# mahyarnajibi/SNIPER

Hardware: AMD Instinct MI355X
Metric: train chips/sec (512x512, R101) (higher is better)
Workload: dtype f16

## Files before the change

include/sniper_hip.h:

```cpp
#ifndef SNIPER_HIP_H
#define SNIPER_HIP_H

#include <stddef.h>
#include <stdint.h>

#ifdef __cplusplus
extern "C" {
#endif

typedef void *sn_stream_t;

enum { SN_OK = 0, SN_ERR_ARG = 1, SN_ERR_HIP = 2, SN_ERR_WORKSPACE = 3, SN_ERR_UNSUPPORTED = 4 };

int sn_version(void);
const char *sn_last_error(void);
int sn_debug_option(const char *name, int value);

int sn_iou_f64(const double *d_boxes, int N, const double *d_query, int K, double *d_out, int mode, sn_stream_t stream);

int sn_chips_num_candidates(int width, int height, int chipsize, int stride);
size_t sn_chips_workspace_bytes(int total_cand, int max_boxes_per_unit);
int sn_chips_generate_batch(const float *d_boxes, const int32_t *d_box_off, const int32_t *d_meta, const int32_t *d_perm,
                            const int32_t *d_cand_off, int U, int max_boxes_per_unit, void *d_mask_ws, float *d_out_chips,
                            int32_t *d_out_ids, int32_t *d_out_count, sn_stream_t stream);
// ... 11 lines not shown

int sn_focus_mask(const float *d_gt, const int32_t *d_ngt, const double *d_crop, const float *d_scale, int B, int G, int F,
                  int feat_stride, int im_h, int im_w, float dc_low, float small_thresh, float dc_high, float *d_mask,
                  sn_stream_t stream);

size_t sn_nms_workspace_bytes(int B, int N);
int sn_nms_batch(const float *d_boxes, const int32_t *d_n, int B, int N, int dim, float thresh, int max_keep, void *d_ws,
                 int32_t *d_keep, int32_t *d_nkeep, sn_stream_t stream);
int sn_nms_host(int *keep_out, int *num_out, const float *boxes_host, int boxes_num, int boxes_dim,
                float nms_overlap_thresh, int device_id);

size_t sn_soft_nms_max_boxes(void);
size_t sn_soft_nms_workspace_bytes(size_t total_rows);
int sn_soft_nms_batch(float *d_boxes, const int32_t *d_off, int P, int max_n, size_t total_rows, float sigma, float Nt,
                      float threshold, int method, void *d_ws, int32_t *d_count, sn_stream_t stream);

int sn_im_prepare(const uint8_t *d_src_bgr, int src_h, int src_w, int crop_x1, int crop_y1, int crop_x2, int crop_y2, double scale,
                  int flip, const double *pixel_means_bgr3, float *d_out, int out_h, int out_w, int32_t *resized_hw2,
                  sn_stream_t stream);
int sn_bbox_decode(const float *d_rois, const float *d_deltas, const float *d_im_info, double *d_boxes, int B, int R,
                   sn_stream_t stream);
int sn_focus_rects_host(const uint8_t *mask_hw, int H, int W, int mode, int32_t *rects_xywh, int cap, int32_t *n_rects);
int sn_focus_chips_host(const float *map_hw, int H, int W, int d, float thresh, int ms, double im_width, double im_height,
                        double cscale, double *chips_xyxy, int max_chips, int32_t *n_chips);
int sn_aggregate_problems_host(const uint64_t *part_rows, const int64_t *lens, const int32_t *part_of_image, const float *range2,
                               int P, int nc, int num_images, float *out_rows, long capacity_rows, int64_t *out_sizes,
                               int64_t *total_rows);
int sn_aggregate_count(const void *d_parts, int P, int nc, int32_t *d_kept, sn_stream_t stream);
int sn_aggregate_scatter(const void *d_parts, int P, int nc, const int32_t *d_dst_off, float *d_out_rows, sn_stream_t stream);
int sn_det_cap_per_image(float *d_rows, const int32_t *d_off, int32_t *d_count, int num_images, int nc, int max_per_image,
                         sn_stream_t stream);
int sn_det_compact(const float *d_scores, const double *d_boxes, const double *h_crops, const double *h_im_wh, float thresh,
                   double delta, int B, int R, int NC, double *d_rows, int32_t *d_counts, sn_stream_t stream);


int sn_conv_fwd(const void *x, const void *w, const float *bias, const void *residual, void *y, int N, int H, int W, int Cin,
                int in_pix_stride, int Cout, int out_pix_stride, int res_pix_stride, int KH, int KW, int stride, int pad, int dil,
                int relu, int out_f32, sn_stream_t stream);
size_t sn_conv_fwd_splitk_workspace_bytes(int N, int H, int W, int Cin, int in_pix_stride, int Cout, int out_pix_stride,
                                          int res_pix_stride, int KH, int KW, int stride, int pad, int dil);
int sn_conv_fwd_splitk(const void *x, const void *w, const float *bias, const void *residual, void *y, int N, int H, int W, int Cin,
                       int in_pix_stride, int Cout, int out_pix_stride, int res_pix_stride, int KH, int KW, int stride, int pad,
                       int dil, int relu, void *ws, size_t ws_bytes, sn_stream_t stream);
int sn_conv_fwd_splitk_f32(const void *x, const void *w, const float *bias, float *y, int N, int H, int W, int Cin, int in_pix_stride,
                           int Cout, int out_pix_stride, int KH, int KW, int stride, int pad, int dil, int relu, void *ws,
                           size_t ws_bytes, sn_stream_t stream);
int sn_conv_fwd_dual_ok(int N, int H, int W, int Cin, int in_pix_stride, int Cout, int out_pix_stride, int res_pix_stride, int KH,
                        int KW, int stride, int pad, int dil, int y2_pix_stride);
int sn_conv_fwd_dual(const void *x, const void *w, const float *bias, const void *residual, void *y, int N, int H, int W, int Cin,
                     int in_pix_stride, int Cout, int out_pix_stride, int res_pix_stride, int KH, int KW, int stride, int pad, int dil,
                     int relu, void *y2, int y2_pix_stride, const float *y2_scale, const float *y2_shift, int y2_relu, void *ws,
                     size_t ws_bytes, sn_stream_t stream);
int sn_conv_tune(int cfg);

int sn_conv_fwd_stats_blocks(int N, int H, int W, int Cin, int in_pix_stride, int Cout, int out_pix_stride, int res_pix_stride,
                             int KH, int KW, int stride, int pad, int dil);
int sn_conv_fwd_stats(const void *x, const void *w, const float *bias, const void *residual, void *y, int N, int H, int W, int Cin,
                      int in_pix_stride, int Cout, int out_pix_stride, int res_pix_stride, int KH, int KW, int stride, int pad,
                      int dil, int relu, float *stats, sn_stream_t stream);
int sn_conv_stem_fwd(const void *xp, const void *w, const float *bias, void *y, int N, int Hp, int Wp, int Ho, int Wo, int Cout,
                     int out_pix_stride, int KH, int KWP, int stride, int relu, int out_f32, sn_stream_t stream);
size_t sn_conv_stem_wgrad_workspace_bytes(int N, int Ho, int Wo, int Cout, int KH, int KWP);
int sn_conv_stem_wgrad(const void *dy, const void *xp, float *dw, int N, int Hp, int Wp, int Ho, int Wo, int Cout, int dy_pix_stride,
                       int KH, int KWP, int stride, void *ws, size_t ws_bytes, sn_stream_t stream);
int sn_conv_dgrad(const void *dy, const void *wt, const void *accumulate, void *dx, int N, int H, int W, int Cin,
                  int dx_pix_stride, int Cout, int dy_pix_stride, int acc_pix_stride, int KH, int KW, int stride, int pad, int dil,
                  int out_f32, sn_stream_t stream);
int sn_conv_dgrad_by_class(int on);
int sn_conv_dgrad_bn_blocks(int N, int H, int W, int Cin, int dx_pix_stride, int Cout, int dy_pix_stride, int acc_pix_stride, int KH,
                            int KW, int stride, int pad, int dil);
int sn_conv_dgrad_bn(const void *dy, const void *wt, const void *accumulate, void *dx, int N, int H, int W, int Cin, int dx_pix_stride,
                     int Cout, int dy_pix_stride, int acc_pix_stride, int KH, int KW, int stride, int pad, int dil, const void *bn_x,
                     int bn_x_pix_stride, const float *bn_scale, const float *bn_shift, const float *bn_mean, int bn_act,
                     float *partials, sn_stream_t stream);
size_t sn_conv_wgrad_workspace_bytes(int N, int H, int W, int Cin, int x_pix_stride, int Cout, int dy_pix_stride, int KH, int KW,
                                     int stride, int pad, int dil);
int sn_conv_wgrad(const void *dy, const void *x, float *dw, int N, int H, int W, int Cin, int x_pix_stride, int Cout,
                  int dy_pix_stride, int KH, int KW, int stride, int pad, int dil, void *ws, size_t ws_bytes, sn_stream_t stream);
typedef struct sn_wgrad_desc {
  const void *dy, *x;
  float *dw;
  int N, H, W, Cin, x_pix_stride, Cout, dy_pix_stride, KH, KW, stride, pad, dil;
} sn_wgrad_desc;
size_t sn_conv_wgrad_batch_workspace_bytes(const sn_wgrad_desc *descs, int n);
int sn_conv_wgrad_batch(const sn_wgrad_desc *descs, int n, void *ws, size_t ws_bytes, sn_stream_t stream);
int sn_conv_wgrad_impl(int impl, int job_steps);
int sn_conv_wgrad_trace(void *buf);
int sn_conv_trace(void *buf);
size_t sn_bias_grad_workspace_bytes(long rows, int C);
int sn_bias_grad(const void *dy, float *db, long rows, int C, int ld, int dtype, void *ws, size_t ws_bytes, sn_stream_t stream);

int sn_pack_stem_input(const float *x_nchw, void *out, int N, int C, int H, int W, int Hp, int Wp, int pad_t, int pad_l,
                       const float *scale, const float *shift, sn_stream_t stream);

size_t sn_bn_workspace_bytes(int M, int C);
int sn_bn_stats(const void *x, int M, int C, int ps, void *ws, sn_stream_t stream);
int sn_bn_finalize(const void *ws, int M, int C, float eps, float momentum, const float *gamma, const float *beta,
                   float *run_mean, float *run_var, float *scale, float *shift, float *save_mean, float *save_invstd,
                   sn_stream_t stream);
int sn_bn_finalize_blocks(const float *partials, int nblk, int M, int C, float eps, float momentum, const float *gamma,
                          const float *beta, float *run_mean, float *run_var, float *scale, float *shift, float *save_mean,
                          float *save_invstd, sn_stream_t stream);
int sn_bn_global_scale_shift(const float *gamma, const float *beta, const float *mean, const float *var, int C, float eps,
                             float *scale, float *shift, sn_stream_t stream);
int sn_bn_apply(const void *x, void *y, int M, int C, int ps_in, int ps_out, const float *scale, const float *shift, int relu,
                sn_stream_t stream);
// ... 253 lines not shown
```

sniper_amd/csrc/common.h:

```cpp
#pragma once
#include <hip/hip_runtime.h>
#include <stdint.h>
#include <stdio.h>
#include <stdlib.h>

#include "../../include/sniper_hip.h"

#define SN_EXPORT extern "C" __attribute__((visibility("default")))

void sn_set_error(const char *fmt, ...);

#define SN_REQUIRE(cond, ...)      \
  do {                             \
    if (!(cond)) {                 \
      sn_set_error(__VA_ARGS__);   \
      return SN_ERR_ARG;           \
    }                              \
  } while (0)

#define SN_CHECK_LAUNCH()                                                      \
  do {                                                                         \
    hipError_t e__ = hipGetLastError();                                        \
    if (e__ != hipSuccess) {                                                   \
      sn_set_error("%s:%d HIP launch failed: %s", __FILE__, __LINE__, hipGetErrorString(e__)); \
      return SN_ERR_HIP;                                                       \
    }                                                                          \
  } while (0)

#define SN_HIP(call)                                                           \
  do {                                                                         \
    hipError_t e__ = (call);                                                   \
    if (e__ != hipSuccess) {                                                   \
      sn_set_error("%s:%d %s: %s", __FILE__, __LINE__, #call, hipGetErrorString(e__)); \
      return SN_ERR_HIP;                                                       \
    }                                                                          \
  } while (0)

hipError_t sn_once_per_device_max_lds(const void *kernel, int bytes);
enum SnDebugOption { SN_OPT_PROPOSAL_FULL_SORT = 0, SN_OPT_NMS_FULL_MASK = 1, SN_OPT_CONV_NO_PERSIST = 2, SN_OPT_SOFTMAX_STRIDED = 3, SN_OPT_COUNT };
int sn_debug_get(SnDebugOption which);

static inline hipStream_t sn_stream(sn_stream_t s) { return (hipStream_t)s; }
static inline int sn_div_up(int a, int b) { return (a + b - 1) / b; }
static inline size_t sn_align(size_t x, size_t a = 256) { return (x + a - 1) / a * a; }

static inline int sn_env_int(const char *name, int dflt) {
  const char *v = getenv(name);
  return v && *v ? atoi(v) : dflt;
}
static inline int sn_conv_out(int in, int k, int stride, int pad, int dil) { return (in + 2 * pad - dil * (k - 1) - 1) / stride + 1; }
static inline int sn_blocks(long total, int cap) {
  const long b = (total + 255) / 256;
  return (int)(b < 1 ? 1 : (b > cap ? cap : b));
}

constexpr int kWave = 64;

typedef _Float16 half_t;
typedef _Float16 half8 __attribute__((ext_vector_type(8)));
typedef _Float16 half4 __attribute__((ext_vector_type(4)));
typedef float floatx4 __attribute__((ext_vector_type(4)));

__device__ __forceinline__ unsigned sn_float_key(float f) {
  const unsigned u = __float_as_uint(f);
  return (u & 0x80000000u) ? ~u : (u | 0x80000000u);
}

int sn_partial_sum(const float *part, int nblk, long n, float *dst, hipStream_t s);

struct SnDiv { unsigned mul, sh, d; };
static inline SnDiv sn_div_make(unsigned d) {
  SnDiv f;
  unsigned s = 0;
  while ((1ull << s) < d) ++s;
  f.mul = (unsigned)((((unsigned long long)1 << 32) * (((unsigned long long)1 << s) - d)) / d + 1);
  f.sh = s;
  f.d = d;
  return f;
}
__device__ __forceinline__ unsigned sn_div(unsigned n, const SnDiv f) { return (__umulhi(n, f.mul) + n) >> f.sh; }
__device__ __forceinline__ unsigned sn_divmod(unsigned n, const SnDiv f, unsigned &rem) {
  const unsigned q = sn_div(n, f);
  rem = n - q * f.d;
  return q;
}
```

sniper_amd/csrc/common.hip:

```cpp
#include "common.h"

#include <stdarg.h>
#include <stdlib.h>
#include <string.h>

#include <atomic>
#include <mutex>
#include <string>
#include <utility>
#include <vector>

static thread_local char g_err[512] = "";

void sn_set_error(const char *fmt, ...) {
  va_list ap;
  va_start(ap, fmt);
  vsnprintf(g_err, sizeof(g_err), fmt, ap);
  va_end(ap);
}

SN_EXPORT const char *sn_last_error(void) { return g_err; }
SN_EXPORT int sn_version(void) { return 100; }

hipError_t sn_once_per_device_max_lds(const void *kernel, int bytes) {
  static std::mutex mu;
  static std::vector<std::pair<const void *, int>> done;
  int dev = 0;
  hipError_t e = hipGetDevice(&dev);
  if (e != hipSuccess) return e;
  std::lock_guard<std::mutex> lock(mu);
  for (const auto &d : done)
    if (d.first == kernel && d.second == dev) return hipSuccess;
  e = hipFuncSetAttribute(kernel, hipFuncAttributeMaxDynamicSharedMemorySize, bytes);
  if (e == hipSuccess) done.emplace_back(kernel, dev);
  return e;
}

static std::atomic<int> g_debug[SN_OPT_COUNT];
static const char *const kDebugNames[SN_OPT_COUNT] = {"proposal_full_sort", "nms_full_mask", "conv_no_persist", "softmax_strided"};
static const char *const kDebugEnv[SN_OPT_COUNT] = {"SNIPER_FULL_SORT", "SNIPER_NMS_FULL", "SNIPER_CONV_NO_PERSIST", "SNIPER_SOFTMAX_STRIDED"};
namespace {
struct DebugInit {
  DebugInit() {
    for (int i = 0; i < SN_OPT_COUNT; ++i) g_debug[i].store(getenv(kDebugEnv[i]) != nullptr ? 1 : 0, std::memory_order_relaxed);
  }
} g_debug_init;
}

int sn_debug_get(SnDebugOption which) { return g_debug[which].load(std::memory_order_relaxed); }

__global__ __launch_bounds__(256) void partial_sum_kernel(const float *__restrict__ part, int nblk, long n, float *__restrict__ dst) {
  const long e = (long)blockIdx.x * 256 + threadIdx.x;
  if (e >= n) return;
  float s = 0.f;
  int k = 0;
  for (; k + 8 <= nblk; k += 8) {
    float v[8];
#pragma unroll
    for (int u = 0; u < 8; ++u) v[u] = part[(size_t)(k + u) * n + e];
#pragma unroll
    for (int u = 0; u < 8; ++u) s += v[u];
  }
  for (; k < nblk; ++k) s += part[(size_t)k * n + e];
  dst[e] += s;
}

int sn_partial_sum(const float *part, int nblk, long n, float *dst, hipStream_t s) {
  hipLaunchKernelGGL(partial_sum_kernel, dim3((unsigned)((n + 255) / 256)), dim3(256), 0, s, part, nblk, n, dst);
  SN_CHECK_LAUNCH();
  return SN_OK;
}

SN_EXPORT int sn_debug_option(const char *name, int value) {
  SN_REQUIRE(name, "sn_debug_option: null name");
  for (int i = 0; i < SN_OPT_COUNT; ++i)
    if (strcmp(name, kDebugNames[i]) == 0) {
      g_debug[i].store(value, std::memory_order_relaxed);
      return SN_OK;
    }
  SN_REQUIRE(false, "sn_debug_option: unknown option '%s'", name);
}
```

sniper_amd/csrc/conv.hip:

```cpp
#include <algorithm>
#include <atomic>

#include "conv_common.h"

#include <stdlib.h>

__device__ __forceinline__ int swz(int row, int chunk) { return chunk ^ ((0x78 >> (2 * ((row >> 2) & 3))) & 3); }

template <int BM, int BN, bool DGRAD>
__global__ __launch_bounds__(256) void conv_igemm_kernel(const ConvParams p) {
  constexpr int BK = 32;
  constexpr int WM = BM / 2, WN = BN / 2;
  constexpr int MI = WM / 16, NI = WN / 16;
  constexpr int AR = BM / 64, BR = BN / 64;
  __shared__ __attribute__((aligned(16))) half_t sA[2][BM * BK];
  __shared__ __attribute__((aligned(16))) half_t sB[2][BN * BK];

  const int tid = threadIdx.x, lane = tid & 63, wave = tid >> 6;
  const int wm = wave >> 1, wn = wave & 1;
  const int m0 = blockIdx.x * BM, n0 = blockIdx.y * BN;
  const int chunk = tid & 3, lrow = tid >> 2;

  int a_base[AR], a_h[AR], a_w[AR];
  bool a_ok[AR];
// ... 73 lines not shown
#pragma unroll
    for (int i = 0; i < MI; ++i) {
      const int r = wm * WM + i * 16 + fr;
      fa[i] = *reinterpret_cast<const half8 *>(&sA[cur][(r * 4 + swz(r, fq)) * 8]);
    }
#pragma unroll
    for (int j = 0; j < NI; ++j) {
      const int r = wn * WN + j * 16 + fr;
      fb[j] = *reinterpret_cast<const half8 *>(&sB[cur][(r * 4 + swz(r, fq)) * 8]);
    }
#pragma unroll
    for (int i = 0; i < MI; ++i)
#pragma unroll
      for (int j = 0; j < NI; ++j) acc[i][j] = __builtin_amdgcn_mfma_f32_16x16x32_f16(fa[i], fb[j], acc[i][j], 0, 0, 0);
    if (kt + 1 < nk) lstore(cur ^ 1);
    __syncthreads();
  }

#pragma unroll
  for (int i = 0; i < MI; ++i) {
#pragma unroll
    for (int r = 0; r < 4; ++r) {
      const int m = m0 + wm * WM + i * 16 + fq * 4 + r;
      if (m >= p.M) continue;
#pragma unroll
      for (int j = 0; j < NI; ++j) {
        const int n = n0 + wn * WN + j * 16 + fr;
        if (n >= p.Nout) continue;
        float v = acc[i][j][r];
        if (p.bias) v += p.bias[n];
        if (p.res) v += (float)p.res[(size_t)m * p.res_ps + n];
        if (p.relu) v = v > 0.f ? v : 0.f;
        if (p.out_f32) reinterpret_cast<float *>(p.y)[(size_t)m * p.out_ps + n] = v;
        else reinterpret_cast<half_t *>(p.y)[(size_t)m * p.out_ps + n] = (half_t)v;
      }
    }
  }
}

static int conv_check(const ConvParams &p, const char *who) {
  SN_REQUIRE(p.x && p.w && p.y, "%s: null pointer", who);
  SN_REQUIRE(p.N > 0 && p.H > 0 && p.W > 0 && p.Ho > 0 && p.Wo > 0 && p.Nout > 0, "%s: bad dims", who);
  SN_REQUIRE(p.Cin > 0 && p.Cin % 8 == 0, "%s: channels per tap must be a multiple of 8 (got %d)", who, p.Cin);
  SN_REQUIRE(p.in_ps % 8 == 0 || (p.in_ps == 4 && p.stride % 2 == 0 && p.KW == 1 && p.pad == 0 && p.W % 2 == 0),
             "%s: source pixel stride must be a multiple of 8 elements (got %d)", who, p.in_ps);
  SN_REQUIRE(p.KH > 0 && p.KW > 0 && p.stride > 0 && p.dil > 0 && p.pad >= 0, "%s: bad kernel geometry", who);
  SN_REQUIRE((long)p.N * p.H * p.W * p.in_ps < (1l << 31) && (long)p.M * p.out_ps < (1l << 31),
             "%s: tensor too large for 32-bit offsets", who);
  return SN_OK;
}

struct ConvPlan {
  int bm, mtiles, ntiles, dma;
  unsigned x_bytes, w_bytes;
  int cls, cls_mc;
};
static std::atomic<int> g_conv_cfg{sn_env_int("SNIPER_CONV_CFG", -1)};
SN_EXPORT int sn_conv_tune(int cfg) {
  SN_REQUIRE(cfg == -1 || cfg == 0 || conv_dma_config(cfg).bm > 0, "sn_conv_tune: no configuration %d", cfg);
  g_conv_cfg.store(cfg, std::memory_order_relaxed);
  return SN_OK;
}

static int conv_dma_choice_balanced(int M, int Nout, int nk, bool dgrad) {
  const long t128 = (long)sn_div_up(M, 128) * sn_div_up(Nout, 128);
  if (t128 >= 3840 && nk >= 8) return 7;
  if (Nout < 128) return nk >= 64 ? 5 : 6;
  if (M < 8192) return (Nout >= 1024 && nk >= 128) ? 4 : 6;
  const int bal = 14, bal_d = 16;
  if (nk <= 1) return 6;
  if (nk >= 16 && (long)sn_div_up(M, 160) * sn_div_up(Nout, 128) <= 320) return 18;
  return dgrad ? bal_d : bal;
}

static std::atomic<int> g_dgrad_by_class{sn_env_int("SNIPER_DGRAD_BY_CLASS", 1)};
SN_EXPORT int sn_conv_dgrad_by_class(int on) {
  g_dgrad_by_class.store(on ? 1 : 0, std::memory_order_relaxed);
  return SN_OK;
}

static ConvPlan conv_plan(const ConvParams &p, bool dgrad, int use_cfg = -1, bool ragged_ok = false) {
  ConvPlan q = {0, 0, 0, 0, 0u, 0u, 0, 0};
  const unsigned long x_bytes = ((unsigned long)p.N * p.H * p.W - 1) * p.in_ps * 2 + (unsigned long)p.Cin * 2;
  const unsigned long w_bytes = (unsigned long)p.Nout * p.KH * p.KW * p.Cin * 2;
  const bool ragged = p.Cin % 64 != 0;
  const int kpt = (p.Cin + 63) / 64;
  if (p.Nout >= 65 && (ragged ? ragged_ok && p.Cin % 8 == 0 : true) && p.in_ps % 8 == 0 && x_bytes <= 0xFFFFFF00ul && w_bytes <= 0xFFFFFF00ul) {
    q.x_bytes = (unsigned)x_bytes;
    q.w_bytes = (unsigned)w_bytes;
    const int forced = g_conv_cfg.load(std::memory_order_relaxed);
    const bool by_class = dgrad && p.stride == 2 && p.dil == 1 && p.Ho % 2 == 0 && p.Wo % 2 == 0 &&
                          g_dgrad_by_class.load(std::memory_order_relaxed) != 0;
    const int nk_full = p.KH * p.KW * kpt;
    const int nk = by_class ? std::max(1, ((p.KH + 1) / 2) * ((p.KW + 1) / 2) * kpt) : nk_full;
    int cfg = use_cfg > 0 ? use_cfg : (forced >= 0 ? forced : conv_dma_choice_balanced(p.M, p.Nout, nk, dgrad));
    if (ragged && cfg > 0) cfg = conv_dma_ragged_cfg(cfg, dgrad);
    if (by_class && cfg == 18 && use_cfg <= 0 && forced < 0) cfg = 16;
    const bool rows16 = !p.out_f32 && !p.out2 && !p.bias && p.out_ps % 8 == 0 && p.Nout % 8 == 0 && (!p.res || p.res_ps % 8 == 0) &&
                        (!p.bn_x || (p.stats && !p.res && p.bn_x_ps % 8 == 0));
    const bool may_persist = !by_class && p.ksplit <= 1 && rows16 && p.KH == 1 && p.KW == 1 && p.stride == 1 && p.pad == 0 &&
                             conv_persist_tiles_per_wg(p.M, p.Nout, 160, 128) > 0;
    if (use_cfg <= 0 && forced < 0 && !ragged && (cfg == 14 || cfg == 16) && may_persist && nk >= 2 && nk <= 16 && sn_debug_get(SN_OPT_CONV_NO_PERSIST) == 0)
      cfg += 10;
    if ((cfg == 24 || cfg == 26) && (!may_persist || nk < 2)) cfg -= 10;
    if (cfg > 0) {
      const ConvDmaConfig c = conv_dma_config(cfg);
      q.dma = cfg;
      q.bm = c.bm;
      q.ntiles = sn_div_up(p.Nout, c.bn);
      const bool cls = by_class && c.bm * c.bn <= 160 * 128 && cfg != 18;
      q.cls = cls ? 1 : 0;
      q.cls_mc = cls ? p.N * (p.Ho / 2) * (p.Wo / 2) : 0;
      q.mtiles = cls ? 4 * sn_div_up(q.cls_mc, c.bm) : sn_div_up(p.M, c.bm);
      return q;
    }
  }
  return q;
}

template <bool DGRAD>
static int conv_launch(const ConvParams &p, hipStream_t s, int use_cfg = -1) {
  const ConvPlan pl = conv_plan(p, DGRAD, use_cfg, !p.stats && !p.out2 && p.ksplit <= 1);
  if (pl.dma) {
    ConvParams q = p;
    q.x_bytes = pl.x_bytes;
    q.w_bytes = pl.w_bytes;
    q.cls = pl.cls;
    q.cls_mc = pl.cls_mc;
    conv_fastdiv_fill(q);
    return conv_dma_launch(q, DGRAD, pl.dma, s);
  }
  SN_REQUIRE(!p.stats, "convolution statistics are emitted by the pipelined kernel only (query sn_conv_fwd_stats_blocks first)");
  if (p.Nout <= 64) {
    dim3 grid(sn_div_up(p.M, 128), sn_div_up(p.Nout, 64));
    hipLaunchKernelGGL((conv_igemm_kernel<128, 64, DGRAD>), grid, dim3(256), 0, s, p);
  } else {
    dim3 grid(sn_div_up(p.M, 128), sn_div_up(p.Nout, 128));
    hipLaunchKernelGGL((conv_igemm_kernel<128, 128, DGRAD>), grid, dim3(256), 0, s, p);
  }
  SN_CHECK_LAUNCH();
  return SN_OK;
}

static void conv_fwd_params(ConvParams &p, const void *x, const void *w, const float *bias, const void *residual, void *y, int N, int H,
                            int W, int Cin, int in_pix_stride, int Cout, int out_pix_stride, int res_pix_stride, int KH, int KW,
                            int stride, int pad, int dil, int relu, int out_f32) {
  p.x = (const half_t *)x; p.w = (const half_t *)w; p.y = y; p.bias = bias; p.res = (const half_t *)residual;
  p.N = N; p.H = H; p.W = W; p.Cin = Cin; p.in_ps = in_pix_stride;
  p.Ho = sn_conv_out(H, KH, stride, pad, dil);
  p.Wo = sn_conv_out(W, KW, stride, pad, dil);
  p.Nout = Cout; p.out_ps = out_pix_stride; p.res_ps = res_pix_stride;
  p.KH = KH; p.KW = KW; p.stride = stride; p.pad = pad; p.dil = dil;
  p.M = N * p.Ho * p.Wo; p.relu = relu; p.out_f32 = out_f32;
}

SN_EXPORT int sn_conv_fwd(const void *x, const void *w, const float *bias, const void *residual, void *y, int N, int H,
                          int W, int Cin, int in_pix_stride, int Cout, int out_pix_stride, int res_pix_stride, int KH,
                          int KW, int stride, int pad, int dil, int relu, int out_f32, sn_stream_t stream) {
  ConvParams p;
  conv_fwd_params(p, x, w, bias, residual, y, N, H, W, Cin, in_pix_stride, Cout, out_pix_stride, res_pix_stride, KH, KW, stride, pad,
                  dil, relu, out_f32);
  if (int rc = conv_check(p, "sn_conv_fwd")) return rc;
  return conv_launch<false>(p, sn_stream(stream));
}

struct SplitPlan { int ksplit; size_t slab_elems; int cfg; };
static SplitPlan conv_split_plan(const ConvParams &p) {
  SplitPlan sp = {1, 0, -1};
  if (p.out_f32 || p.stats) return sp;
  ConvPlan pl = conv_plan(p, false);
  if (!pl.dma) return sp;
  ConvDmaConfig c = conv_dma_config(pl.dma);
  const int nk = p.KH * p.KW * (p.Cin / 64);
  if (c.bm * c.bn > 160 * 128) {
    if (g_conv_cfg.load(std::memory_order_relaxed) >= 0 || p.M >= 8192 || nk < 32) return sp;
    sp.cfg = 5;
    pl = conv_plan(p, false, sp.cfg);
    c = conv_dma_config(pl.dma);
    if (!pl.dma || c.bm * c.bn > 160 * 128) return SplitPlan{1, 0, -1};
  }
  const long tiles = (long)pl.mtiles * pl.ntiles;
  if (nk < 8 || tiles > 256 || (tiles >= 160 && nk < 64)) return SplitPlan{1, 0, -1};
  int ks = (int)std::min<long>(std::min<long>(nk / 4, (448 + tiles - 1) / tiles), tiles <= 16 ? 16 : 8);
  if (ks < 2) return SplitPlan{1, 0, -1};
  sp.ksplit = ks;
  sp.slab_elems = (size_t)p.M * p.Nout;
  return sp;
}

__global__ __launch_bounds__(256) void splitk_reduce_kernel(const float *__restrict__ slab, int ksplit, size_t stride, long M, int Nout,
                                                            const float *__restrict__ bias, const half_t *__restrict__ res, int res_ps,
                                                            half_t *__restrict__ out, int out_ps, int relu,
                                                            half_t *__restrict__ out2, int out2_ps, const float *__restrict__ o2_scale,
                                                            const float *__restrict__ o2_shift, int o2_relu, int out_f32) {
  const int cpr = (Nout + 7) >> 3;
  const long total = M * cpr;
  const bool vec = !out_f32 && (Nout & 7) == 0 && (out_ps & 7) == 0 && (!res || (res_ps & 7) == 0);
  for (long i = (long)blockIdx.x * blockDim.x + threadIdx.x; i < total; i += (long)gridDim.x * blockDim.x) {
    const long m = i / cpr;
    const int n = (int)(i - m * cpr) * 8;
    if (!vec) {
      for (int r = 0; r < 8 && n + r < Nout; ++r) {
        float a = 0.f;
        for (int z = 0; z < ksplit; ++z) a += slab[(size_t)z * stride + (size_t)m * Nout + n + r];
        if (bias) a += bias[n + r];
        if (res) a += (float)res[(size_t)m * res_ps + n + r];
        if (relu && a < 0.f) a = 0.f;
        if (out_f32) reinterpret_cast<float *>(out)[(size_t)m * out_ps + n + r] = a;
        else out[(size_t)m * out_ps + n + r] = (half_t)a;
      }
      continue;
    }
    float v[8] = {0.f, 0.f, 0.f, 0.f, 0.f, 0.f, 0.f, 0.f};
    for (int z = 0; z < ksplit; ++z) {
      const float *sp = slab + (size_t)z * stride + (size_t)m * Nout + n;
      const float4 a = *reinterpret_cast<const float4 *>(sp), b = *reinterpret_cast<const float4 *>(sp + 4);
      v[0] += a.x; v[1] += a.y; v[2] += a.z; v[3] += a.w; v[4] += b.x; v[5] += b.y; v[6] += b.z; v[7] += b.w;
    }
    if (bias) {
#pragma unroll
      for (int r = 0; r < 8; ++r) v[r] += bias[n + r];
    }
    if (res) {
      const half8 rv = *reinterpret_cast<const half8 *>(res + (size_t)m * res_ps + n);
#pragma unroll
      for (int r = 0; r < 8; ++r) v[r] += (float)rv[r];
    }
    half8 o;
// ... 73 lines not shown
static bool conv_dual_ok(const ConvParams &p, int y2_pix_stride) {
  if (p.Ho <= 0 || p.Wo <= 0 || p.out_f32 || p.Nout % 8 != 0 || p.out_ps % 8 != 0 || (p.res && p.res_ps % 8 != 0) || y2_pix_stride % 8 != 0)
    return false;
  return conv_plan(p, false).dma != 0;
}

SN_EXPORT int sn_conv_fwd_dual_ok(int N, int H, int W, int Cin, int in_pix_stride, int Cout, int out_pix_stride, int res_pix_stride,
                                  int KH, int KW, int stride, int pad, int dil, int y2_pix_stride) {
  ConvParams p;
  conv_fwd_params(p, nullptr, nullptr, nullptr, nullptr, nullptr, N, H, W, Cin, in_pix_stride, Cout, out_pix_stride, res_pix_stride, KH,
                  KW, stride, pad, dil, 0, 0);
  if (res_pix_stride % 8 != 0) return 0;
  return conv_dual_ok(p, y2_pix_stride) ? 1 : 0;
}

SN_EXPORT int sn_conv_fwd_dual(const void *x, const void *w, const float *bias, const void *residual, void *y, int N, int H, int W,
                               int Cin, int in_pix_stride, int Cout, int out_pix_stride, int res_pix_stride, int KH, int KW, int stride,
                               int pad, int dil, int relu, void *y2, int y2_pix_stride, const float *y2_scale, const float *y2_shift,
                               int y2_relu, void *ws, size_t ws_bytes, sn_stream_t stream) {
  ConvParams p;
  conv_fwd_params(p, x, w, bias, residual, y, N, H, W, Cin, in_pix_stride, Cout, out_pix_stride, res_pix_stride, KH, KW, stride, pad,
                  dil, relu, 0);
  if (int rc = conv_check(p, "sn_conv_fwd_dual")) return rc;
  SN_REQUIRE(y2 && y2_scale && y2_shift && conv_dual_ok(p, y2_pix_stride),
             "sn_conv_fwd_dual: the layer does not take the 16-byte pipelined epilogue (query sn_conv_fwd_dual_ok)");
  const SplitPlan sp = conv_split_plan(p);
  if (sp.ksplit > 1 && ws && ws_bytes >= (size_t)sp.ksplit * sp.slab_elems * sizeof(float))
    return conv_splitk_run(p, sp, ws, 0, (half_t *)y2, y2_pix_stride, y2_scale, y2_shift, y2_relu, sn_stream(stream));
  p.out2 = (half_t *)y2; p.out2_ps = y2_pix_stride; p.o2_scale = y2_scale; p.o2_shift = y2_shift; p.o2_relu = y2_relu;
  return conv_launch<false>(p, sn_stream(stream));
}

SN_EXPORT int sn_conv_fwd_stats_blocks(int N, int H, int W, int Cin, int in_pix_stride, int Cout, int out_pix_stride,
                                       int res_pix_stride, int KH, int KW, int stride, int pad, int dil) {
  ConvParams p;
  conv_fwd_params(p, nullptr, nullptr, nullptr, nullptr, nullptr, N, H, W, Cin, in_pix_stride, Cout, out_pix_stride, res_pix_stride, KH,
                  KW, stride, pad, dil, 0, 0);
  if (p.Ho <= 0 || p.Wo <= 0 || Cout % 4 != 0 || out_pix_stride % 4 != 0 || (res_pix_stride % 4) != 0) return 0;
  const ConvPlan pl = conv_plan(p, false);
  return pl.bm ? pl.mtiles : 0;
}

SN_EXPORT int sn_conv_fwd_stats(const void *x, const void *w, const float *bias, const void *residual, void *y, int N, int H, int W,
                                int Cin, int in_pix_stride, int Cout, int out_pix_stride, int res_pix_stride, int KH, int KW,
                                int stride, int pad, int dil, int relu, float *stats, sn_stream_t stream) {
  ConvParams p;
  conv_fwd_params(p, x, w, bias, residual, y, N, H, W, Cin, in_pix_stride, Cout, out_pix_stride, res_pix_stride, KH, KW, stride, pad,
                  dil, relu, 0);
  if (int rc = conv_check(p, "sn_conv_fwd_stats")) return rc;
  SN_REQUIRE(stats && Cout % 4 == 0 && out_pix_stride % 4 == 0 && (!residual || res_pix_stride % 4 == 0),
             "sn_conv_fwd_stats: statistics need 8-byte aligned output rows (query sn_conv_fwd_stats_blocks)");
  p.stats = stats;
  return conv_launch<false>(p, sn_stream(stream));
}

SN_EXPORT int sn_conv_stem_fwd(const void *xp, const void *w, const float *bias, void *y, int N, int Hp, int Wp, int Ho, int Wo,
                               int Cout, int out_pix_stride, int KH, int KWP, int stride, int relu, int out_f32,
                               sn_stream_t stream) {
  ConvParams p;
  p.x = (const half_t *)xp; p.w = (const half_t *)w; p.y = y; p.bias = bias; p.res = nullptr;
  p.N = N; p.H = Hp; p.W = Wp; p.Cin = 4 * KWP; p.in_ps = 4;
  p.Ho = Ho; p.Wo = Wo; p.Nout = Cout; p.out_ps = out_pix_stride; p.res_ps = 0;
  p.KH = KH; p.KW = 1; p.stride = stride; p.pad = 0; p.dil = 1;
  p.M = N * Ho * Wo; p.relu = relu; p.out_f32 = out_f32;
  SN_REQUIRE((Ho - 1) * stride + KH <= Hp && (Wo - 1) * stride + KWP <= Wp, "sn_conv_stem_fwd: padded input too small");
  SN_REQUIRE(stride % 2 == 0 && Wp % 2 == 0 && KWP % 2 == 0, "sn_conv_stem_fwd: 16-byte alignment needs even stride/pitch");
  if (int rc = conv_check(p, "sn_conv_stem_fwd")) return rc;
  return conv_launch<false>(p, sn_stream(stream));
}

static void conv_dgrad_params(ConvParams &p, const void *dy, const void *wt, const void *accumulate, void *dx, int N, int H, int W,
                              int Cin, int dx_pix_stride, int Cout, int dy_pix_stride, int acc_pix_stride, int KH, int KW, int stride,
                              int pad, int dil, int out_f32) {
  const int Ho = sn_conv_out(H, KH, stride, pad, dil), Wo = sn_conv_out(W, KW, stride, pad, dil);
  p.x = (const half_t *)dy; p.w = (const half_t *)wt; p.y = dx; p.bias = nullptr; p.res = (const half_t *)accumulate;
  p.N = N; p.H = Ho; p.W = Wo; p.Cin = Cout; p.in_ps = dy_pix_stride;
  p.Ho = H; p.Wo = W; p.Nout = Cin; p.out_ps = dx_pix_stride; p.res_ps = acc_pix_stride;
  p.KH = KH; p.KW = KW; p.stride = stride; p.pad = pad; p.dil = dil;
  p.M = N * H * W; p.relu = 0; p.out_f32 = out_f32;
}

SN_EXPORT int sn_conv_dgrad(const void *dy, const void *wt, const void *accumulate, void *dx, int N, int H, int W,
                            int Cin, int dx_pix_stride, int Cout, int dy_pix_stride, int acc_pix_stride, int KH, int KW,
                            int stride, int pad, int dil, int out_f32, sn_stream_t stream) {
  ConvParams p;
  conv_dgrad_params(p, dy, wt, accumulate, dx, N, H, W, Cin, dx_pix_stride, Cout, dy_pix_stride, acc_pix_stride, KH, KW, stride, pad,
                    dil, out_f32);
  if (int rc = conv_check(p, "sn_conv_dgrad")) return rc;
  return conv_launch<true>(p, sn_stream(stream));
}

SN_EXPORT int sn_conv_dgrad_bn_blocks(int N, int H, int W, int Cin, int dx_pix_stride, int Cout, int dy_pix_stride,
                                      int acc_pix_stride, int KH, int KW, int stride, int pad, int dil) {
  ConvParams p;
  conv_dgrad_params(p, nullptr, nullptr, nullptr, nullptr, N, H, W, Cin, dx_pix_stride, Cout, dy_pix_stride, acc_pix_stride, KH, KW,
                    stride, pad, dil, 0);
  if (p.H <= 0 || p.W <= 0 || Cin % 4 != 0 || dx_pix_stride % 4 != 0 || acc_pix_stride % 4 != 0) return 0;
  const ConvPlan pl = conv_plan(p, true);
  return pl.bm ? pl.mtiles : 0;
}

SN_EXPORT int sn_conv_dgrad_bn(const void *dy, const void *wt, const void *accumulate, void *dx, int N, int H, int W, int Cin,
                               int dx_pix_stride, int Cout, int dy_pix_stride, int acc_pix_stride, int KH, int KW, int stride, int pad,
                               int dil, const void *bn_x, int bn_x_pix_stride, const float *bn_scale, const float *bn_shift,
                               const float *bn_mean, int bn_act, float *partials, sn_stream_t stream) {
  ConvParams p;
// ... 339 lines not shown
```

sniper_amd/csrc/conv_common.h:

```cpp
#pragma once
#include <atomic>
#include "common.h"

struct ConvParams {
  const half_t *x;
  const half_t *w;
  void *y;
  const float *bias;
  const half_t *res;
  int N, H, W;
  int Cin, in_ps;
  int Ho, Wo;
  int Nout, out_ps, res_ps;
  int KH, KW, stride, pad, dil;
  int M;
  int relu, out_f32;
  unsigned x_bytes, w_bytes;
  const half_t *bn_x = nullptr;
  const float *bn_scale = nullptr, *bn_shift = nullptr, *bn_mean = nullptr;
  int bn_x_ps = 0, bn_act = 0;
  unsigned fda_mul = 1, fda_sh = 0, fdb_mul = 1, fdb_sh = 0;
  int rows_img = 1, row_len = 1;
  int cls = 0, cls_mc = 0;
  int ksplit = 1, ksplit_grid = 0;
  long ksplit_stride = 0;
  unsigned long long *trace = nullptr;
  half_t *out2 = nullptr;
  const float *o2_scale = nullptr, *o2_shift = nullptr;
  int out2_ps = 0, o2_relu = 0;
  int tiles_per_wg = 1;
  float *stats = nullptr;
};


static inline void conv_fastdiv_fill(ConvParams &p) {
  p.rows_img = p.cls ? (p.Ho / 2) * (p.Wo / 2) : p.Ho * p.Wo;
  p.row_len = p.cls ? p.Wo / 2 : p.Wo;
  const SnDiv a = sn_div_make((unsigned)p.rows_img), b = sn_div_make((unsigned)p.row_len);
  p.fda_mul = a.mul; p.fda_sh = a.sh;
  p.fdb_mul = b.mul; p.fdb_sh = b.sh;
}

typedef __attribute__((address_space(3))) void *lds_ptr_t;
typedef short short4v __attribute__((vector_size(8)));

__device__ __forceinline__ void dma16(__amdgpu_buffer_rsrc_t rsrc, half_t *dst, unsigned voff) {
  __builtin_amdgcn_raw_ptr_buffer_load_lds(rsrc, (lds_ptr_t)dst, 16, voff, 0, 0, 0);
}
template <int N>
__device__ __forceinline__ void wait_vmcnt() {
  asm volatile("s_waitcnt vmcnt(%0)" ::"n"(N) : "memory");
}
__device__ __forceinline__ half8 tr_frag(const half_t *img, int off, int second) {
  typedef __attribute__((address_space(3))) short4v *lds_v4;
  union { short4v s[2]; half8 h; } u;
  u.s[0] = __builtin_amdgcn_ds_read_tr16_b64_v4i16((lds_v4)(img + off));
  u.s[1] = __builtin_amdgcn_ds_read_tr16_b64_v4i16((lds_v4)(img + off + second));
  return u.h;
}

struct ConvDmaConfig { int bm, bn, threads, stages, lds_bytes; };
constexpr int kConvPersistWgs = 512;
static inline int conv_persist_tiles_per_wg(int M, int Nout, int bm, int bn) {
  if (M % bm || Nout % bn) return 0;
  const long mt = M / bm, nt = Nout / bn, tiles = mt * nt;
  if (mt % 8 || tiles < 2 * kConvPersistWgs || tiles % kConvPersistWgs) return 0;
  return (int)(tiles / kConvPersistWgs);
}
constexpr int kConvDmaConfigs = 26;
ConvDmaConfig conv_dma_config(int cfg);
int conv_dma_launch(const ConvParams &p, bool dgrad, int cfg, hipStream_t s);
void conv_dma_set_trace(unsigned long long *buf);
int conv_dma_ragged_cfg(int cfg, bool dgrad);
int conv_dma_ragged_launch(const ConvParams &p, bool dgrad, int cfg, hipStream_t s);

struct WgradParams {
  const half_t *dy;
  const half_t *x;
  float *dw;
  int N, H, W, Ho, Wo, Cin, Cout, dy_ps, x_ps;
  int KH, KW, stride, pad, dil;
  int units_per_split;
  float *slab;
  size_t slab_stride;
  int gx, gy, gz, per_xcd;
};

__device__ __forceinline__ bool wgrad_block(const WgradParams &p, int &bx, int &by, int &bz) {
  const int b = blockIdx.x;
  const int item = (b & 7) * p.per_xcd + (b >> 3);
  const int tiles = p.gx * p.gy;
  if (item >= tiles * p.gz) return false;
  bz = item / tiles;
  const int r = item - bz * tiles;
  by = r / p.gx;
  bx = r - by * p.gx;
  return true;
}
static inline unsigned wgrad_grid(WgradParams &p, int gx, int gy, int gz) {
  p.gx = gx; p.gy = gy; p.gz = gz;
  p.per_xcd = (gx * gy * gz + 7) / 8;
  return 8u * (unsigned)p.per_xcd;
}

struct WgradProblem {
  const half_t *dy, *x;
  float *dw, *slab;
  size_t slab_stride;
  int N, H, W, Ho, Wo, Cin, Cout, dy_ps, x_ps, KH, KW, stride, pad, dil;
  int gx, gy, taps, splits, units_per_split, cpr, nunits, item0;
};
constexpr int kWgradMaxProblems = 24;
struct WgradBatch {
  int n, total_items, per_xcd, reserved;
  int xcd_start[9];
  int reserved2;
  unsigned long long *trace;
  WgradProblem p[kWgradMaxProblems];
};
bool wgrad_ps_ok(const WgradParams &p);
size_t wgrad_ps_plan(const WgradParams *ps, int n, WgradBatch &tab, void *ws, bool allow_split, int na);
int wgrad_ps_launch(const WgradBatch &tab, hipStream_t s, int na);
void wgrad_ps_set_job_steps(int steps);
void wgrad_ps_set_trace(unsigned long long *buf);
```

Before: 992.6.

## Add weight-resident streaming conv kernel for narrow-output forward layers

Adds a persistent forward-conv kernel for layers with at most 64 output channels. It preloads the whole weight tensor and bias into LDS once per workgroup, then streams activations from global memory straight into registers through a four-deep ring of buffer loads feeding MFMA. The planner routes qualifying large-M forward convs to it by default, with an env/debug switch to disable it. This aims to cut the repeated weight staging and low utilization of the existing narrow-N path, at the cost of LDS-limited occupancy and a new code path.

Result: no change. 991.8 (-0.1%).

```diff
diff --git a/include/sniper_hip.h b/include/sniper_hip.h
--- a/include/sniper_hip.h
+++ b/include/sniper_hip.h
@@ -87,6 +87,10 @@
                      int relu, void *y2, int y2_pix_stride, const float *y2_scale, const float *y2_shift, int y2_relu, void *ws,
                      size_t ws_bytes, sn_stream_t stream);
 int sn_conv_tune(int cfg);
+int sn_conv_stream_ok(int N, int H, int W, int Cin, int in_pix_stride, int Cout, int out_pix_stride, int res_pix_stride, int KH,
+                      int KW, int stride, int pad, int dil, int flags);
+int sn_conv_stem_stream_ok(int N, int Hp, int Wp, int Ho, int Wo, int Cout, int out_pix_stride, int KH, int KWP, int stride,
+                           int out_f32);
 
 int sn_conv_fwd_stats_blocks(int N, int H, int W, int Cin, int in_pix_stride, int Cout, int out_pix_stride, int res_pix_stride,
                              int KH, int KW, int stride, int pad, int dil);
diff --git a/sniper_amd/csrc/common.h b/sniper_amd/csrc/common.h
--- a/sniper_amd/csrc/common.h
+++ b/sniper_amd/csrc/common.h
@@ -37,7 +37,7 @@
   } while (0)
 
 hipError_t sn_once_per_device_max_lds(const void *kernel, int bytes);
-enum SnDebugOption { SN_OPT_PROPOSAL_FULL_SORT = 0, SN_OPT_NMS_FULL_MASK = 1, SN_OPT_CONV_NO_PERSIST = 2, SN_OPT_SOFTMAX_STRIDED = 3, SN_OPT_COUNT };
+enum SnDebugOption { SN_OPT_PROPOSAL_FULL_SORT = 0, SN_OPT_NMS_FULL_MASK = 1, SN_OPT_CONV_NO_PERSIST = 2, SN_OPT_SOFTMAX_STRIDED = 3, SN_OPT_CONV_NO_STREAM = 4, SN_OPT_COUNT };
 int sn_debug_get(SnDebugOption which);
 
 static inline hipStream_t sn_stream(sn_stream_t s) { return (hipStream_t)s; }
diff --git a/sniper_amd/csrc/common.hip b/sniper_amd/csrc/common.hip
--- a/sniper_amd/csrc/common.hip
+++ b/sniper_amd/csrc/common.hip
@@ -37,8 +37,8 @@
 }
 
 static std::atomic<int> g_debug[SN_OPT_COUNT];
-static const char *const kDebugNames[SN_OPT_COUNT] = {"proposal_full_sort", "nms_full_mask", "conv_no_persist", "softmax_strided"};
-static const char *const kDebugEnv[SN_OPT_COUNT] = {"SNIPER_FULL_SORT", "SNIPER_NMS_FULL", "SNIPER_CONV_NO_PERSIST", "SNIPER_SOFTMAX_STRIDED"};
+static const char *const kDebugNames[SN_OPT_COUNT] = {"proposal_full_sort", "nms_full_mask", "conv_no_persist", "softmax_strided", "conv_no_stream"};
+static const char *const kDebugEnv[SN_OPT_COUNT] = {"SNIPER_FULL_SORT", "SNIPER_NMS_FULL", "SNIPER_CONV_NO_PERSIST", "SNIPER_SOFTMAX_STRIDED", "SNIPER_CONV_NO_STREAM"};
 namespace {
 struct DebugInit {
   DebugInit() {
diff --git a/sniper_amd/csrc/conv.hip b/sniper_amd/csrc/conv.hip
--- a/sniper_amd/csrc/conv.hip
+++ b/sniper_amd/csrc/conv.hip
@@ -149,12 +149,13 @@
 
 struct ConvPlan {
   int bm, mtiles, ntiles, dma;
+  int stream;
   unsigned x_bytes, w_bytes;
   int cls, cls_mc;
 };
 static std::atomic<int> g_conv_cfg{sn_env_int("SNIPER_CONV_CFG", -1)};
 SN_EXPORT int sn_conv_tune(int cfg) {
-  SN_REQUIRE(cfg == -1 || cfg == 0 || conv_dma_config(cfg).bm > 0, "sn_conv_tune: no configuration %d", cfg);
+  SN_REQUIRE(cfg == -1 || cfg == 0 || cfg == kConvStreamCfg || conv_dma_config(cfg).bm > 0, "sn_conv_tune: no configuration %d", cfg);
   g_conv_cfg.store(cfg, std::memory_order_relaxed);
   return SN_OK;
 }
@@ -176,16 +177,23 @@
   return SN_OK;
 }
 
+constexpr int kConvStreamMinM = 16384, kConvStreamMinMNarrow = 131072;
 static ConvPlan conv_plan(const ConvParams &p, bool dgrad, int use_cfg = -1, bool ragged_ok = false) {
-  ConvPlan q = {0, 0, 0, 0, 0u, 0u, 0, 0};
+  ConvPlan q = {0, 0, 0, 0, 0, 0u, 0u, 0, 0};
   const unsigned long x_bytes = ((unsigned long)p.N * p.H * p.W - 1) * p.in_ps * 2 + (unsigned long)p.Cin * 2;
   const unsigned long w_bytes = (unsigned long)p.Nout * p.KH * p.KW * p.Cin * 2;
+  const int tune = g_conv_cfg.load(std::memory_order_relaxed);
+  if (!dgrad && use_cfg <= 0 && (tune == -1 || tune == kConvStreamCfg) && sn_debug_get(SN_OPT_CONV_NO_STREAM) == 0 && conv_stream_can(p) &&
+      (tune == kConvStreamCfg || p.M >= (p.Nout < 32 ? kConvStreamMinMNarrow : kConvStreamMinM))) {
+    q.stream = 1;
+    return q;
+  }
   const bool ragged = p.Cin % 64 != 0;
   const int kpt = (p.Cin + 63) / 64;
   if (p.Nout >= 65 && (ragged ? ragged_ok && p.Cin % 8 == 0 : true) && p.in_ps % 8 == 0 && x_bytes <= 0xFFFFFF00ul && w_bytes <= 0xFFFFFF00ul) {
     q.x_bytes = (unsigned)x_bytes;
     q.w_bytes = (unsigned)w_bytes;
-    const int forced = g_conv_cfg.load(std::memory_order_relaxed);
+    const int forced = tune == kConvStreamCfg ? -1 : tune;
     const bool by_class = dgrad && p.stride == 2 && p.dil == 1 && p.Ho % 2 == 0 && p.Wo % 2 == 0 &&
                           g_dgrad_by_class.load(std::memory_order_relaxed) != 0;
     const int nk_full = p.KH * p.KW * kpt;
@@ -227,6 +235,7 @@
     conv_fastdiv_fill(q);
     return conv_dma_launch(q, DGRAD, pl.dma, s);
   }
+  if (pl.stream) return conv_stream_launch(p, s);
   SN_REQUIRE(!p.stats, "convolution statistics are emitted by the pipelined kernel only (query sn_conv_fwd_stats_blocks first)");
   if (p.Nout <= 64) {
     dim3 grid(sn_div_up(p.M, 128), sn_div_up(p.Nout, 64));
@@ -270,7 +279,8 @@
   ConvDmaConfig c = conv_dma_config(pl.dma);
   const int nk = p.KH * p.KW * (p.Cin / 64);
   if (c.bm * c.bn > 160 * 128) {
-    if (g_conv_cfg.load(std::memory_order_relaxed) >= 0 || p.M >= 8192 || nk < 32) return sp;
+    const int tune = g_conv_cfg.load(std::memory_order_relaxed);
+    if ((tune >= 0 && tune != kConvStreamCfg) || p.M >= 8192 || nk < 32) return sp;
     sp.cfg = 5;
     pl = conv_plan(p, false, sp.cfg);
     c = conv_dma_config(pl.dma);
@@ -450,6 +460,31 @@
              "sn_conv_fwd_stats: statistics need 8-byte aligned output rows (query sn_conv_fwd_stats_blocks)");
   p.stats = stats;
   return conv_launch<false>(p, sn_stream(stream));
+}
+
+SN_EXPORT int sn_conv_stream_ok(int N, int H, int W, int Cin, int in_pix_stride, int Cout, int out_pix_stride, int res_pix_stride,
+                                int KH, int KW, int stride, int pad, int dil, int flags) {
+  ConvParams p;
+  const half_t *some = reinterpret_cast<const half_t *>(16);
+  conv_fwd_params(p, nullptr, nullptr, nullptr, (flags & 1) ? some : nullptr, nullptr, N, H, W, Cin, in_pix_stride, Cout, out_pix_stride,
+                  res_pix_stride, KH, KW, stride, pad, dil, 0, (flags & 2) ? 1 : 0);
+  if (flags & 12) return 0;
+  if (N <= 0 || H <= 0 || W <= 0 || Cin <= 0 || Cout <= 0 || p.Ho <= 0 || p.Wo <= 0 || Cin % 8 != 0 || in_pix_stride % 8 != 0 || KH <= 0 || KW <= 0 ||
+      stride <= 0 || dil <= 0 || pad < 0)
+    return 0;
+  return conv_plan(p, false, -1, true).stream;
+}
+
+SN_EXPORT int sn_conv_stem_stream_ok(int N, int Hp, int Wp, int Ho, int Wo, int Cout, int out_pix_stride, int KH, int KWP, int stride,
+                                     int out_f32) {
+  if (N <= 0 || Hp <= 0 || Wp <= 0 || Ho <= 0 || Wo <= 0 || Cout <= 0 || KH <= 0 || KWP <= 0 || stride <= 0 || stride % 2 || Wp % 2 || KWP % 2) return 0;
+  ConvParams p;
+  p.x = nullptr; p.w = nullptr; p.y = nullptr; p.bias = nullptr; p.res = nullptr;
+  p.N = N; p.H = Hp; p.W = Wp; p.Cin = 4 * KWP; p.in_ps = 4;
+  p.Ho = Ho; p.Wo = Wo; p.Nout = Cout; p.out_ps = out_pix_stride; p.res_ps = 0;
+  p.KH = KH; p.KW = 1; p.stride = stride; p.pad = 0; p.dil = 1;
+  p.M = N * Ho * Wo; p.relu = 0; p.out_f32 = out_f32;
+  return conv_plan(p, false, -1, true).stream;
 }
 
 SN_EXPORT int sn_conv_stem_fwd(const void *xp, const void *w, const float *bias, void *y, int N, int Hp, int Wp, int Ho, int Wo,
diff --git a/sniper_amd/csrc/conv_common.h b/sniper_amd/csrc/conv_common.h
--- a/sniper_amd/csrc/conv_common.h
+++ b/sniper_amd/csrc/conv_common.h
@@ -74,6 +74,10 @@
 int conv_dma_ragged_cfg(int cfg, bool dgrad);
 int conv_dma_ragged_launch(const ConvParams &p, bool dgrad, int cfg, hipStream_t s);
 
+constexpr int kConvStreamCfg = 30;
+bool conv_stream_can(const ConvParams &p);
+int conv_stream_launch(const ConvParams &p, hipStream_t s);
+
 struct WgradParams {
   const half_t *dy;
   const half_t *x;
diff --git a/sniper_amd/csrc/conv_stream.hip b/sniper_amd/csrc/conv_stream.hip
--- /dev/null
+++ b/sniper_amd/csrc/conv_stream.hip
@@ -0,0 +1,197 @@
+#include <algorithm>
+
+#include "conv_common.h"
+
+typedef unsigned uint4v __attribute__((ext_vector_type(4)));
+
+constexpr int kStreamThreads = 512;
+constexpr int kStreamTile = 128;
+constexpr int kStreamWgs = 512;
+constexpr int kStreamDepth = 4;
+constexpr size_t kStreamLdsBudget = 80 * 1024;
+constexpr unsigned kStreamInvalid = 0xFFFFFF00u;
+
+template <int NT>
+__device__ __forceinline__ int stream_chan(int t, int i) {
+  if ((t | 1) < NT) return 32 * (t >> 1) + 8 * (i >> 2) + 4 * (t & 1) + (i & 3);
+  return 16 * t + i;
+}
+
+template <int NT, int KC>
+__global__ __launch_bounds__(kStreamThreads, 4) void conv_stream_kernel(const ConvParams p) {
+  constexpr int D = kStreamDepth;
+  extern __shared__ __attribute__((aligned(16))) unsigned char smem[];
+  const int tid = threadIdx.x, lane = tid & 63, wave = tid >> 6;
+  const int fr = lane & 15, fq = lane >> 4;
+  const int taps = p.KH * p.KW, kpt = p.Cin >> 5, nkb = taps * kpt;
+  const int wrow = taps * p.Cin;
+
+  const int pieces = nkb * NT * 64;
+  for (int e = tid; e < pieces; e += kStreamThreads) {
+    const int l = e & 63, tk = e >> 6, kb = tk / NT, t = tk - kb * NT;
+    const int c = stream_chan<NT>(t, l & 15);
+    *reinterpret_cast<half8 *>(smem + (size_t)e * 16) = *reinterpret_cast<const half8 *>(p.w + (size_t)c * wrow + kb * 32 + 8 * (l >> 4));
+  }
+  float *sbias = reinterpret_cast<float *>(smem + (size_t)pieces * 16);
+  if (tid < NT * 16) sbias[tid] = p.bias ? p.bias[tid] : 0.f;
+  __syncthreads();
+
+  const int ntiles = (p.M + kStreamTile - 1) / kStreamTile;
+  const int mine = (int)blockIdx.x < ntiles ? (ntiles - 1 - (int)blockIdx.x) / (int)gridDim.x + 1 : 0;
+  const int tstep = gridDim.x;
+  const int spt = kpt / KC, S = taps * spt;
+  const long T = (long)mine * S;
+  const __amdgpu_buffer_rsrc_t rx = __builtin_amdgcn_make_buffer_rsrc(const_cast<half_t *>(p.x), 0, (int)p.x_bytes, 0x00020000);
+  const SnDiv fda = {p.fda_mul, p.fda_sh, (unsigned)p.rows_img}, fdb = {p.fdb_mul, p.fdb_sh, (unsigned)p.row_len};
+
+  int l_tile = blockIdx.x, l_kh = 0, l_kw = 0, l_cb = 0;
+  bool l_ok;
+  unsigned l_base;
+  int l_iy, l_ix;
+  auto set_rows = [&](int tile) {
+    const long m = ((long)tile * 8 + wave) * 16 + fr;
+    l_ok = m < p.M;
+    unsigned rem;
+    const unsigned img = sn_divmod(l_ok ? (unsigned)m : 0u, fda, rem);
+    unsigned ox;
+    const unsigned oy = sn_divmod(rem, fdb, ox);
+    l_base = img * (unsigned)(p.H * p.W);
+    l_iy = (int)oy * p.stride - p.pad;
+    l_ix = (int)ox * p.stride - p.pad;
+  };
+  set_rows(l_tile);
+  auto issue = [&](uint4v(&buf)[KC]) {
+    const int sy = l_iy + l_kh * p.dil, sx = l_ix + l_kw * p.dil;
+    const bool ok = l_ok && (unsigned)sy < (unsigned)p.H && (unsigned)sx < (unsigned)p.W;
+    unsigned off = ((l_base + (unsigned)(sy * p.W + sx)) * (unsigned)p.in_ps + (unsigned)(l_cb * KC * 32 + fq * 8)) * 2u;
+    off = ok ? off : kStreamInvalid;
+#pragma unroll
+    for (int k = 0; k < KC; ++k) buf[k] = __builtin_amdgcn_raw_buffer_load_b128(rx, (int)(off + 64u * k), 0, 0);
+    if (++l_cb == spt) {
+      l_cb = 0;
+      if (++l_kw == p.KW) {
+        l_kw = 0;
+        if (++l_kh == p.KH) {
+          l_kh = 0;
+          l_tile += tstep;
+          set_rows(l_tile);
+        }
+      }
+    }
+  };
+
+  int c_tile = blockIdx.x, c_s = 0;
+  floatx4 acc[NT];
+  half_t *const y = reinterpret_cast<half_t *>(p.y);
+  auto epilogue = [&]() {
+    const long m = ((long)c_tile * 8 + wave) * 16 + fr;
+    const bool ok = m < p.M;
+    half_t *const row = y + (size_t)(ok ? m : 0) * p.out_ps;
+#pragma unroll
+    for (int u = 0; u < NT / 2; ++u) {
+      const floatx4 b0 = *reinterpret_cast<const floatx4 *>(sbias + 32 * u + 8 * fq), b1 = *reinterpret_cast<const floatx4 *>(sbias + 32 * u + 8 * fq + 4);
+      half8 o;
+#pragma unroll
+      for (int r = 0; r < 4; ++r) {
+        float v0 = acc[2 * u][r] + b0[r], v1 = acc[2 * u + 1][r] + b1[r];
+        if (p.relu) { v0 = v0 > 0.f ? v0 : 0.f; v1 = v1 > 0.f ? v1 : 0.f; }
+        o[r] = (half_t)v0;
+        o[4 + r] = (half_t)v1;
+      }
+      if (ok) *reinterpret_cast<half8 *>(row + 32 * u + 8 * fq) = o;
+    }
+    if constexpr (NT & 1) {
+      constexpr int t = NT - 1;
+      const floatx4 b = *reinterpret_cast<const floatx4 *>(sbias + 16 * t + 4 * fq);
+      union { half4 h; int w[2]; } mine4, other;
+#pragma unroll
+      for (int r = 0; r < 4; ++r) {
+        float v = acc[t][r] + b[r];
+        if (p.relu) v = v > 0.f ? v : 0.f;
+        mine4.h[r] = (half_t)v;
+      }
+      other.w[0] = __shfl_xor(mine4.w[0], 16);
+      other.w[1] = __shfl_xor(mine4.w[1], 16);
+      if (ok && !(fq & 1)) {
+        half8 o;
+#pragma unroll
+        for (int r = 0; r < 4; ++r) { o[r] = mine4.h[r]; o[4 + r] = other.h[r]; }
+        *reinterpret_cast<half8 *>(row + 16 * t + 4 * fq) = o;
+      }
+    }
+  };
+  auto compute = [&](const uint4v(&buf)[KC]) {
+    if (c_s == 0) {
+#pragma unroll
+      for (int t = 0; t < NT; ++t) acc[t] = floatx4{0.f, 0.f, 0.f, 0.f};
+    }
+    const unsigned char *img = smem + ((size_t)c_s * KC * NT * 64 + lane) * 16;
+#pragma unroll
+    for (int k = 0; k < KC; ++k) {
+      union { uint4v u; half8 h; } b;
+      b.u = buf[k];
+#pragma unroll
+      for (int t = 0; t < NT; ++t) {
+        const half8 a = *reinterpret_cast<const half8 *>(img + (size_t)(k * NT + t) * 1024);
+        acc[t] = __builtin_amdgcn_mfma_f32_16x16x32_f16(a, b.h, acc[t], 0, 0, 0);
+      }
+    }
+    if (++c_s == S) {
+      epilogue();
+      c_s = 0;
+      c_tile += tstep;
+    }
+  };
+
+  uint4v ring[D][KC];
+#pragma unroll
+  for (int d = 0; d < D; ++d) issue(ring[d]);
+  for (long g = 0; g < T; g += D) {
+#pragma unroll
+    for (int d = 0; d < D; ++d) {
+      compute(ring[d]);
+      issue(ring[d]);
+    }
+  }
+}
+
+size_t conv_stream_lds_bytes(const ConvParams &p) { return (size_t)p.Nout * p.KH * p.KW * p.Cin * 2 + (size_t)p.Nout * 4; }
+
+bool conv_stream_can(const ConvParams &p) {
+  if (p.Nout > 64 || p.Nout % 16 != 0 || p.Cin % 32 != 0 || p.out_ps % 8 != 0) return false;
+  if (!(p.in_ps % 8 == 0 || (p.in_ps == 4 && p.stride % 2 == 0 && p.KW == 1 && p.pad == 0 && p.W % 2 == 0))) return false;
+  if (p.res || p.stats || p.out2 || p.out_f32 || p.ksplit > 1 || p.bn_x) return false;
+  const unsigned long x_bytes = ((unsigned long)p.N * p.H * p.W - 1) * p.in_ps * 2 + (unsigned long)p.Cin * 2;
+  if (x_bytes > kStreamInvalid) return false;
+  return conv_stream_lds_bytes(p) <= kStreamLdsBudget;
+}
+
+template <int NT, int KC>
+static int stream_launch_one(const ConvParams &p, hipStream_t s) {
+  const int lds = (int)conv_stream_lds_bytes(p);
+  const void *fn = reinterpret_cast<const void *>(&conv_stream_kernel<NT, KC>);
+  SN_HIP(sn_once_per_device_max_lds(fn, (int)kStreamLdsBudget));
+  const int ntiles = sn_div_up(p.M, kStreamTile);
+  hipLaunchKernelGGL((conv_stream_kernel<NT, KC>), dim3((unsigned)std::min(ntiles, kStreamWgs)), dim3(kStreamThreads), lds, s, p);
+  SN_CHECK_LAUNCH();
+  return SN_OK;
+}
+
+template <int KC>
+static int stream_launch_kc(const ConvParams &p, hipStream_t s) {
+  switch (p.Nout / 16) {
+    case 1: return stream_launch_one<1, KC>(p, s);
+    case 2: return stream_launch_one<2, KC>(p, s);
+    case 3: return stream_launch_one<3, KC>(p, s);
+    default: return stream_launch_one<4, KC>(p, s);
+  }
+}
+
+int conv_stream_launch(const ConvParams &p, hipStream_t s) {
+  SN_REQUIRE(conv_stream_can(p), "conv_stream_launch: the layer does not qualify");
+  ConvParams q = p;
+  q.x_bytes = (unsigned)(((unsigned long)p.N * p.H * p.W - 1) * p.in_ps * 2 + (unsigned long)p.Cin * 2);
+  q.cls = 0;
+  conv_fastdiv_fill(q);
+  return (p.Cin / 32) % 2 == 0 ? stream_launch_kc<2>(q, s) : stream_launch_kc<1>(q, s);
+}
```
